# megvii-research/Far3D

Measured on AMD Instinct MI355X. Metric: samples/sec (7-cam frame) end-to-end @ VoV-99 640x960, higher is better.
Workload: dtype bf16x3; 1 GPU; BASELINE configs[1]: 7 cameras 3x640x960, VoV-99, A=1544 queries (644 learned + 644 adaptive + 256 propagated), 2312 self-attn keys, 6 decoder layers, streaming memory on, ego motion on; proposals=topk, fused_rows=True, parallelism=single GPU, weights=seeded random (far3d_amd.weights.init_state_dict, seed 0)

## Files before the change

far3d_amd/csrc/norm.hip:

```cpp
#include "common.hpp"

__device__ __forceinline__ float wave_sum(float v) {
#pragma unroll
  for (int o = 32; o >= 1; o >>= 1) v += __shfl_xor(v, o);
  return v;
}

template <int MAXV>
__global__ __launch_bounds__(256) void layernorm_kernel(const float* __restrict__ x, const float* __restrict__ gamma,
                                                        const float* __restrict__ beta, float* __restrict__ y, int rows,
                                                        int C, int ldx, int ldy, float eps, int act,
                                                        const float* __restrict__ add, int lda, void* __restrict__ y2,
                                                        int ldy2, int y2_dt, void* __restrict__ yb, int ldyb, int yb_dt,
                                                        const int* __restrict__ out_rows) {
  const int lane = threadIdx.x & 63;
  const int row = blockIdx.x * 4 + (threadIdx.x >> 6);
  if (row >= rows) return;
  const int orow = out_rows ? out_rows[row] : row;
  const float* xr = x + (long)row * ldx;
  float4 v[MAXV];
  float s = 0.f;
#pragma unroll
  for (int i = 0; i < MAXV; ++i) {
    const int c = (lane + 64 * i) * 4;
// ... 279 lines not shown
    hipLaunchKernelGGL(ese_apply_kernel<float>, dim3((unsigned)blocks), dim3(256), 0, st, (const float*)x, gate,
                       (const float*)identity, (float*)y, total4, C, HW, ldx, x_img_stride, ldi, i_img_stride, ldy, y_img_stride, chan_sums, N * C);
  else if (dt == FAR3D_DT_BF16_PAIR)
    hipLaunchKernelGGL(ese_apply_kernel<pair_t>, dim3((unsigned)blocks), dim3(256), 0, st, (const pair_t*)x, gate,
                       (const pair_t*)identity, (pair_t*)y, total4, C, HW, ldx, x_img_stride, ldi, i_img_stride, ldy, y_img_stride, chan_sums, N * C);
  else
    hipLaunchKernelGGL(ese_apply_kernel<bf16_t>, dim3((unsigned)blocks), dim3(256), 0, st, (const bf16_t*)x, gate,
                       (const bf16_t*)identity, (bf16_t*)y, total4, C, HW, ldx, x_img_stride, ldi, i_img_stride, ldy, y_img_stride, chan_sums, N * C);
  FAR3D_CHECK_LAUNCH("far3d_ese_nhwc");
  return FAR3D_OK;
}

template <typename T> struct Vec8;
template <> struct Vec8<bf16_t> {
  struct Raw { uint4 a; };
  static __device__ __forceinline__ Raw ldraw(const bf16_t* p) { Raw r; r.a = *reinterpret_cast<const uint4*>(p); return r; }
  static __device__ __forceinline__ void cvt(const Raw& q, float (&v)[8]) {
    const uint4 r = q.a;
    v[0] = __uint_as_float(r.x << 16); v[1] = __uint_as_float(r.x & 0xffff0000u); v[2] = __uint_as_float(r.y << 16); v[3] = __uint_as_float(r.y & 0xffff0000u);
    v[4] = __uint_as_float(r.z << 16); v[5] = __uint_as_float(r.z & 0xffff0000u); v[6] = __uint_as_float(r.w << 16); v[7] = __uint_as_float(r.w & 0xffff0000u);
  }
  static __device__ __forceinline__ void ld(const bf16_t* p, float (&v)[8]) {
    const uint4 r = *reinterpret_cast<const uint4*>(p);
    v[0] = __uint_as_float(r.x << 16); v[1] = __uint_as_float(r.x & 0xffff0000u); v[2] = __uint_as_float(r.y << 16); v[3] = __uint_as_float(r.y & 0xffff0000u);
    v[4] = __uint_as_float(r.z << 16); v[5] = __uint_as_float(r.z & 0xffff0000u); v[6] = __uint_as_float(r.w << 16); v[7] = __uint_as_float(r.w & 0xffff0000u);
  }
  static __device__ __forceinline__ void st(bf16_t* p, const float (&v)[8]) {
    *reinterpret_cast<uint4*>(p) = make_uint4(pack_bf16x2(v[0], v[1]), pack_bf16x2(v[2], v[3]), pack_bf16x2(v[4], v[5]), pack_bf16x2(v[6], v[7]));
  }
  static __device__ __forceinline__ void round(float (&v)[8]) {
#pragma unroll
    for (int e = 0; e < 8; e += 2) { const uint32_t q = pack_bf16x2(v[e], v[e + 1]); v[e] = __uint_as_float(q << 16); v[e + 1] = __uint_as_float(q & 0xffff0000u); }
  }
};
template <> struct Vec8<pair_t> {
  struct Raw { uint4 h, l; };
  static __device__ __forceinline__ Raw ldraw(const pair_t* p) {
    Raw r;
    r.h = *reinterpret_cast<const uint4*>(p);
    r.l = *reinterpret_cast<const uint4*>(reinterpret_cast<const bf16_t*>(p) + 32);
    return r;
  }
  static __device__ __forceinline__ void cvt(const Raw& q, float (&v)[8]) {
    float h[8], l[8];
    Vec8<bf16_t>::Raw a, b;
    a.a = q.h; b.a = q.l;
    Vec8<bf16_t>::cvt(a, h);
    Vec8<bf16_t>::cvt(b, l);
#pragma unroll
    for (int e = 0; e < 8; ++e) v[e] = h[e] + l[e];
  }
  static __device__ __forceinline__ void ld(const pair_t* p, float (&v)[8]) {
    float h[8], l[8];
    Vec8<bf16_t>::ld(reinterpret_cast<const bf16_t*>(p), h);
    Vec8<bf16_t>::ld(reinterpret_cast<const bf16_t*>(p) + 32, l);
#pragma unroll
    for (int e = 0; e < 8; ++e) v[e] = h[e] + l[e];
  }
  static __device__ __forceinline__ void split(const float (&v)[8], uint4& h, uint4& l) {
    uint2 h0, l0, h1, l1;
    split4f(v[0], v[1], v[2], v[3], h0, l0);
    split4f(v[4], v[5], v[6], v[7], h1, l1);
    h = make_uint4(h0.x, h0.y, h1.x, h1.y); l = make_uint4(l0.x, l0.y, l1.x, l1.y);
  }
  static __device__ __forceinline__ void st(pair_t* p, const float (&v)[8]) {
    uint4 h, l;
    split(v, h, l);
    *reinterpret_cast<uint4*>(p) = h;
    *reinterpret_cast<uint4*>(reinterpret_cast<bf16_t*>(p) + 32) = l;
  }
  static __device__ __forceinline__ void round(float (&v)[8]) {
    uint4 h, l;
    split(v, h, l);
    const uint32_t hh[4] = {h.x, h.y, h.z, h.w}, ll[4] = {l.x, l.y, l.z, l.w};
#pragma unroll
    for (int e = 0; e < 4; ++e) {
      v[2 * e] = __uint_as_float(hh[e] << 16) + __uint_as_float(ll[e] << 16);
      v[2 * e + 1] = __uint_as_float(hh[e] & 0xffff0000u) + __uint_as_float(ll[e] & 0xffff0000u);
    }
  }
};

struct EseFusedParams {
  const void* x; const void* idn; void* y; void* pooled;
  const float* gate; long long* sums;
  int N, H, W, C, ldx, ldi, ldy, ldp, Hp, Wp, DB;
  long xs, is, ys, ps;
};

template <typename T, bool POOL>
__global__ __launch_bounds__(256) __attribute__((amdgpu_waves_per_eu(4, 8))) void ese_fused_kernel(EseFusedParams P) {
  const int n = blockIdx.y, tid = threadIdx.x, C = P.C;
  const int b = blockIdx.x, cq = C / 8;
  const int HW = P.H * P.W;
  const int stride = P.DB * 256;
  const int i0 = b * 256 + tid;
  const int cg = i0 % cq, pstep = stride / cq;
  const int co = chan_off<T>(cg * 8);
  const T* x = reinterpret_cast<const T*>(P.x) + (long)n * P.xs + co;
  const T* idn = P.idn ? reinterpret_cast<const T*>(P.idn) + (long)n * P.is + co : nullptr;
  T* y = P.y ? reinterpret_cast<T*>(P.y) + (long)n * P.ys + co : nullptr;
  int pix = i0 / cq;
  float g[8];
  {
    const float4 g0 = *reinterpret_cast<const float4*>(P.gate + (long)n * C + cg * 8), g1 = *reinterpret_cast<const float4*>(P.gate + (long)n * C + cg * 8 + 4);
    g[0] = g0.x; g[1] = g0.y; g[2] = g0.z; g[3] = g0.w; g[4] = g1.x; g[5] = g1.y; g[6] = g1.z; g[7] = g1.w;
  }
  float xv[8], dv[8];
  if (y && pix < HW) {
    Vec8<T>::ld(x + (long)pix * P.ldx, xv);
    if (idn) Vec8<T>::ld(idn + (long)pix * P.ldi, dv);
  }
  for (int i = i0; i < C; i += stride) P.sums[(long)n * C + i] = 0;
  if (y) {
    for (; pix < HW; pix += pstep) {
      const int nxt = pix + pstep;
      float xn[8], dn[8];
      if (nxt < HW) {
        Vec8<T>::ld(x + (long)nxt * P.ldx, xn);
        if (idn) Vec8<T>::ld(idn + (long)nxt * P.ldi, dn);
      }
#pragma unroll
      for (int e = 0; e < 8; ++e) xv[e] = idn ? ese_mul_add(xv[e], g[e], dv[e]) : ese_mul(xv[e], g[e]);
      Vec8<T>::st(y + (long)pix * P.ldy, xv);
#pragma unroll
      for (int e = 0; e < 8; ++e) { xv[e] = xn[e]; dv[e] = dn[e]; }
    }
  }
  if constexpr (POOL) {
    T* pd = reinterpret_cast<T*>(P.pooled) + (long)n * P.ps + co;
    const int HWp = P.Hp * P.Wp;
    for (int q = i0 / cq; q < HWp; q += pstep) {
      const int oy = q / P.Wp, ox = q - oy * P.Wp;
      float m[8];
#pragma unroll
      for (int e = 0; e < 8; ++e) m[e] = -INFINITY;
#pragma unroll 1
      for (int ky = 0; ky < 3; ++ky) {
        const int iy = min(oy * 2 + ky, P.H - 1);
        typename Vec8<T>::Raw tv[3], td[3];
#pragma unroll
        for (int kx = 0; kx < 3; ++kx) {
          const long pp = (long)iy * P.W + min(ox * 2 + kx, P.W - 1);
          tv[kx] = Vec8<T>::ldraw(x + pp * P.ldx);
          if (idn) td[kx] = Vec8<T>::ldraw(idn + pp * P.ldi);
        }
#pragma unroll
        for (int kx = 0; kx < 3; ++kx) {
          float v[8], d[8];
          Vec8<T>::cvt(tv[kx], v);
          if (idn) Vec8<T>::cvt(td[kx], d);
#pragma unroll
          for (int e = 0; e < 8; ++e) v[e] = idn ? ese_mul_add(v[e], g[e], d[e]) : ese_mul(v[e], g[e]);
          Vec8<T>::round(v);
#pragma unroll
          for (int e = 0; e < 8; ++e) m[e] = fmaxf(m[e], v[e]);
        }
      }
      Vec8<T>::st(pd + (long)q * P.ldp, m);
    }
  }
}

extern "C" int far3d_ese_fused_nhwc(const void* x, int dt, const float* fcw, const float* fcb, const void* identity, void* y, void* pooled,
                                    float* gate, int N, int H, int W, int C, int ldx, long x_img_stride, int ldi,
                                    long i_img_stride, int ldy, long y_img_stride, int Hp, int Wp, int ldp, long p_img_stride,
                                    long long* chan_sums, void* stream) {
  FAR3D_CHECK_ARG(x && fcw && fcb && gate && chan_sums && (y || pooled), "far3d_ese_fused_nhwc: null pointer argument (y or pooled must be given)");
  FAR3D_CHECK_ARG(dt == FAR3D_DT_BF16 || dt == FAR3D_DT_BF16_PAIR, "far3d_ese_fused_nhwc: bf16 or pair-stored maps (the fixed-point channel sums describe those)");
  FAR3D_CHECK_ARG(N > 0 && H > 0 && W > 0 && C > 0 && C <= 1024 && C % (dt == FAR3D_DT_BF16_PAIR ? 32 : 8) == 0, "far3d_ese_fused_nhwc: bad sizes (C=%d)", C);
  auto al = [](const void* p) { return ((uintptr_t)p % 16) == 0; };
  FAR3D_CHECK_ARG(al(x) && ldx % 8 == 0 && x_img_stride % 8 == 0 && (!identity || (al(identity) && ldi % 8 == 0 && i_img_stride % 8 == 0)) &&
                  (!y || (al(y) && ldy % 8 == 0 && y_img_stride % 8 == 0)) && (!pooled || (al(pooled) && ldp % 8 == 0 && p_img_stride % 8 == 0)) && al(gate),
                  "far3d_ese_fused_nhwc: pointers and strides must be multiples of 16 bytes");
  if (pooled) {
    int eh = (H - 3 + 1) / 2 + 1; if ((eh - 1) * 2 >= H) --eh;
    int ew = (W - 3 + 1) / 2 + 1; if ((ew - 1) * 2 >= W) --ew;
    FAR3D_CHECK_ARG(Hp == eh && Wp == ew, "far3d_ese_fused_nhwc: pooled size %dx%d != ceil-mode size %dx%d", Hp, Wp, eh, ew);
  }
  hipStream_t st = (hipStream_t)stream;
  hipLaunchKernelGGL(ese_gate_kernel, dim3((C + 15) / 16, N), dim3(256), 0, st, (const float*)nullptr, fcw, fcb, gate, C, 1.f / ((float)H * W), 0,
                     (const long long*)chan_sums);
  EseFusedParams P;
  P.x = x; P.idn = identity; P.y = y; P.pooled = pooled; P.gate = gate; P.sums = chan_sums;
  P.N = N; P.H = H; P.W = W; P.C = C; P.ldx = ldx; P.ldi = ldi; P.ldy = ldy; P.ldp = ldp; P.Hp = Hp; P.Wp = Wp;
  P.xs = x_img_stride; P.is = i_img_stride; P.ys = y_img_stride; P.ps = p_img_stride;
  const int cq = C / 8;
  int unit = 1;
  while ((256 * unit) % cq) ++unit;
  const long items = (long)(y ? H * W : Hp * Wp) * cq;
  long db = (items + 4 * 256 - 1) / (4 * 256);
  if (db > 1200) db = 1200;
  db = (db + unit - 1) / unit * unit;
  P.DB = (int)db;
  dim3 grid((unsigned)P.DB, (unsigned)N);
  if (dt == FAR3D_DT_BF16_PAIR) {
    if (pooled) hipLaunchKernelGGL((ese_fused_kernel<pair_t, true>), grid, dim3(256), 0, st, P);
    else hipLaunchKernelGGL((ese_fused_kernel<pair_t, false>), grid, dim3(256), 0, st, P);
  } else {
    if (pooled) hipLaunchKernelGGL((ese_fused_kernel<bf16_t, true>), grid, dim3(256), 0, st, P);
    else hipLaunchKernelGGL((ese_fused_kernel<bf16_t, false>), grid, dim3(256), 0, st, P);
  }
  FAR3D_CHECK_LAUNCH("far3d_ese_fused_nhwc");
  return FAR3D_OK;
}

__global__ __launch_bounds__(256) void gn_stats_kernel(const float* __restrict__ part, float* __restrict__ stat, int C,
                                                       int groups, float inv_cnt, float eps, int nparts) {
  __shared__ float2 cs[1024];
  const int n = blockIdx.x, cpg = C / groups;
  const float2* src = reinterpret_cast<const float2*>(part) + (long)n * nparts * C;
  float2 sm[4];
  sum_parts<4>(src, nparts, C, threadIdx.x, 256, sm);
#pragma unroll
  for (int j = 0; j < 4; ++j)
    if (threadIdx.x + j * 256 < C) cs[threadIdx.x + j * 256] = sm[j];
  __syncthreads();
  for (int g = threadIdx.x; g < groups; g += 256) {
    float s = 0.f, q = 0.f;
    for (int c = g * cpg; c < (g + 1) * cpg; ++c) { s += cs[c].x; q += cs[c].y; }
    const float mean = s * inv_cnt;
    const float var = fmaxf(q * inv_cnt - mean * mean, 0.f);
    stat[2 * ((long)n * groups + g)] = mean;
    stat[2 * ((long)n * groups + g) + 1] = 1.f / sqrtf(var + eps);
  }
}

template <typename T>
__global__ __launch_bounds__(256) void gn_apply_kernel(const T* __restrict__ x, const float* __restrict__ stat,
                                                       const float* __restrict__ gamma, const float* __restrict__ beta,
                                                       T* __restrict__ y, long total4, int C, int groups, int HW, int relu) {
  const int cq = C / 4, cpg = C / groups;
  for (long i = (long)blockIdx.x * blockDim.x + threadIdx.x; i < total4; i += (long)gridDim.x * blockDim.x) {
    const int c = (int)(i % cq) * 4;
// ... 94 lines not shown
```

far3d_amd/csrc/stem.hip:

```cpp
#include "igemm_kernels.hpp"

__global__ __launch_bounds__(256) __attribute__((amdgpu_waves_per_eu(4, 8))) void stem_conv_kernel(const float* __restrict__ img, const bf16_t* __restrict__ w, const float* __restrict__ bias,
                                                        bf16_t* __restrict__ y, int N, int H, int W, int Ho, int Wo, int ldy, long y_img_stride,
                                                        int tiles_x, int ntiles, int relu) {
  constexpr int RS = 144;
  __shared__ __attribute__((aligned(16))) unsigned char smem[4 * 32 * RS];
  const int lane = threadIdx.x & 63, wv = threadIdx.x >> 6, l31 = lane & 31, hi = lane >> 5;
  unsigned char* my = smem + wv * 32 * RS;
  u32x4_t af[2][2];
#pragma unroll
  for (int i = 0; i < 2; ++i)
#pragma unroll
    for (int h = 0; h < 2; ++h) af[i][h] = *reinterpret_cast<const u32x4_t*>(w + (long)(i * 32 + l31) * 32 + h * 16 + hi * 8);
  int kinfo[16];
#pragma unroll
  for (int s = 0; s < 16; ++s) {
    const int k = (s >> 3) * 16 + hi * 8 + (s & 7);
    const int tap = (k * 11) >> 5, c = k - 3 * tap;
    const int dy = (tap * 11) >> 5, dx = tap - 3 * dy;
    kinfo[s] = ((c * H + dy) * W + dx) | (dy << 24) | (dx << 26) | ((k >= 27 ? 1 : 0) << 28);
  }
  auto gather = [&](int t, float (&v)[16]) __attribute__((always_inline)) {
    const int tx = t % tiles_x, r = t / tiles_x, oy = r % Ho, n = r / Ho;
    const int ox = tx * 32 + l31;
    const int iy0 = 2 * oy - 1, ix0 = 2 * ox - 1;
    const float* base = img + ((long)n * 3 * H + iy0) * W + ix0;
#pragma unroll
    for (int s = 0; s < 16; ++s) {
      const int iy = iy0 + ((kinfo[s] >> 24) & 3), ix = ix0 + ((kinfo[s] >> 26) & 3);
      const bool ok = ox < Wo && !(kinfo[s] >> 28) && iy >= 0 && iy < H && ix >= 0 && ix < W;
      v[s] = ok ? base[kinfo[s] & 0xffffff] : 0.f;
    }
  };
  const int wstride = gridDim.x * 4;
  int t = blockIdx.x * 4 + wv;
  for (; t < ntiles; t += wstride) {
    float cur[16];
    gather(t, cur);
    u32x4_t bf0, bf1;
    bf0.x = pack_bf16x2(cur[0], cur[1]); bf0.y = pack_bf16x2(cur[2], cur[3]); bf0.z = pack_bf16x2(cur[4], cur[5]); bf0.w = pack_bf16x2(cur[6], cur[7]);
    bf1.x = pack_bf16x2(cur[8], cur[9]); bf1.y = pack_bf16x2(cur[10], cur[11]); bf1.z = pack_bf16x2(cur[12], cur[13]); bf1.w = pack_bf16x2(cur[14], cur[15]);
    f32x16_t acc[2];
#pragma unroll
    for (int i = 0; i < 2; ++i) {
#pragma unroll
      for (int r = 0; r < 16; ++r) acc[i][r] = 0.f;
      mma<bf16_t>(acc[i], af[i][0], bf0);
      mma<bf16_t>(acc[i], af[i][1], bf1);
    }
#pragma unroll
    for (int i = 0; i < 2; ++i)
#pragma unroll
      for (int q = 0; q < 4; ++q) {
        const float4 b4 = bias ? *reinterpret_cast<const float4*>(bias + i * 32 + 8 * q + 4 * hi) : make_float4(0.f, 0.f, 0.f, 0.f);
        float v0 = acc[i][4 * q] + b4.x, v1 = acc[i][4 * q + 1] + b4.y, v2 = acc[i][4 * q + 2] + b4.z, v3 = acc[i][4 * q + 3] + b4.w;
        if (relu) { v0 = fmaxf(v0, 0.f); v1 = fmaxf(v1, 0.f); v2 = fmaxf(v2, 0.f); v3 = fmaxf(v3, 0.f); }
        *reinterpret_cast<uint2*>(my + l31 * RS + (i * 32 + 8 * q + 4 * hi) * 2) = make_uint2(pack_bf16x2(v0, v1), pack_bf16x2(v2, v3));
      }
    __builtin_amdgcn_wave_barrier();
    asm volatile("s_waitcnt lgkmcnt(0)" ::: "memory");
    const int tx = t % tiles_x, r = t / tiles_x, oy = r % Ho, n = r / Ho;
    bf16_t* yrow = y + (long)n * y_img_stride + ((long)oy * Wo + tx * 32) * ldy;
#pragma unroll
    for (int it = 0; it < 4; ++it) {
      const int px = it * 8 + (lane >> 3), ch = lane & 7;
      const uint4 v = *reinterpret_cast<const uint4*>(my + px * RS + ch * 16);
      if (tx * 32 + px < Wo) *reinterpret_cast<uint4*>(yrow + (long)px * ldy + ch * 8) = v;
    }
    asm volatile("s_waitcnt lgkmcnt(0)" ::: "memory");
    __builtin_amdgcn_wave_barrier();
  }
}

extern "C" int far3d_stem_conv(const float* img, const void* w, const float* bias, void* y, int N, int H, int W, int ldy, long y_img_stride,
                               int act, void* stream) {
  FAR3D_CHECK_ARG(img && w && y, "far3d_stem_conv: null pointer argument");
  FAR3D_CHECK_ARG(N > 0 && H > 1 && W > 1 && (long)3 * H * W < (1L << 24), "far3d_stem_conv: bad image size N=%d H=%d W=%d (3*H*W < 2^24)", N, H, W);
  FAR3D_CHECK_ARG(act == ACT_NONE || act == ACT_RELU, "far3d_stem_conv: activation none or ReLU");
  FAR3D_CHECK_ARG(((uintptr_t)y % 16) == 0 && ((uintptr_t)w % 16) == 0 && ldy >= 64 && ldy % 8 == 0 && y_img_stride % 8 == 0,
                  "far3d_stem_conv: y / w must be 16-byte aligned, pixel stride a multiple of 8 elements (>= 64)");
  const int Ho = (H - 1) / 2 + 1, Wo = (W - 1) / 2 + 1;
  const int tiles_x = (Wo + 31) / 32, ntiles = N * Ho * tiles_x;
  int blocks = (ntiles + 3) / 4;
  if (blocks > 4096) blocks = 4096;
  hipLaunchKernelGGL(stem_conv_kernel, dim3((unsigned)blocks), dim3(256), 0, (hipStream_t)stream, img, (const bf16_t*)w, bias, (bf16_t*)y, N, H, W, Ho, Wo,
                     ldy, y_img_stride, tiles_x, ntiles, act == ACT_RELU ? 1 : 0);
  FAR3D_CHECK_LAUNCH("far3d_stem_conv");
  return FAR3D_OK;
}
```

far3d_amd/engine.py:

```python
import fnmatch
import functools
import math
import os

import torch
import torch.nn.functional as F

from . import lib as _lib
from . import ops, weights
from .synth import level_starts

PRECISIONS = {
    "bf16": dict(act=torch.bfloat16, value=torch.bfloat16, dec=torch.bfloat16),
    "fp32": dict(act=torch.float32, value=torch.float32, dec=torch.float32),
    "bf16_fp32dec": dict(act=torch.bfloat16, value=torch.bfloat16, dec=torch.float32),
    "bf16_fp32val": dict(act=torch.bfloat16, value=torch.float32, dec=torch.float32),
    "bf16x3": dict(act=torch.bfloat16, pair=True, value=torch.float32, dec=torch.float32, mma="bf16x3", dec_mma=None),
    "bf16x3_all": dict(act=torch.bfloat16, pair=True, value=torch.float32, dec=torch.float32, mma="bf16x3", dec_mma="bf16x3"),
    "bf16x3_2d1": dict(act=torch.bfloat16, pair=True, value=torch.float32, dec=torch.float32, mma="bf16x3", dec_mma=None,
                       single_bf16=("roi[123].*", "depth.*")),
    "bf16x3_f32act": dict(act=torch.float32, value=torch.float32, dec=torch.float32, mma="bf16x3", dec_mma=None),
}


# ... 301 lines not shown
                                     (self.cfg.get("proposal_capacity"), self.cfg["proposal_cap"]))

    def act_from_nchw(self, x):
        y = x.permute(0, 2, 3, 1).contiguous()
        return ops.pair_from_float(y) if self.pair else y.to(self.prec["act"])

    def act_to_nchw(self, y):
        y = ops.pair_to_float(y) if (self.pair and y.dtype == torch.bfloat16) else y.float()
        return y.permute(0, 3, 1, 2).contiguous()

    def _buf(self, key, shape, dtype):
        key = (self._par,) + tuple(key)
        b = self._bufs.get(key)
        if b is None or tuple(b.shape) != tuple(shape) or b.dtype != dtype:
            b = torch.empty(shape, dtype=dtype, device=self.dev)
            self._bufs[key] = b
        return b

    @_with_tile_tables
    def backbone(self, img, keep_stage2=True):
        act, spec, cs, pair = self.prec["act"], self.spec, self.cs, self.pair
        N = img.shape[0]
        Lb = spec["layer_per_block"]
        scratch = self._buf(("ese_scratch",), (ops.ese_scratch_floats(N, max(spec["stage_out_ch"])),), torch.float32)
        esums = None
        if act == torch.bfloat16:
            ek = (self._par, "esums", N)
            esums = self._bufs.get(ek)
            if esums is None:
                esums = self._bufs[ek] = torch.zeros((N, max(spec["stage_out_ch"])), dtype=torch.int64, device=self.dev)
        if esums is not None and not torch.cuda.is_current_stream_capturing():
            esums.zero_()
        egate = self._buf(("ese_gate", N), (N * max(spec["stage_out_ch"]),), torch.float32) if esums is not None else None
        if act == torch.bfloat16 and not pair:
            x = ops.stem_conv(img, self.bb["stem1"], act="relu")
        else:
            x = ops.stem_im2col(img, act, pair=pair)
            x = ops.conv2d_nhwc(x, self.bb["stem1"], act="relu")
        x = ops.conv2d_nhwc(x, self.bb["stem2"], act="relu")
        H, W = self.bb["stem3"].out_hw(x.shape[1], x.shape[2])
        in_ch = spec["stem"][2]
        outs = []
        stage_in = None
        pooled_by_ese = False
        next_cat = None
        for si, blocks in enumerate(self.bb["stages"]):
            sc, oc = spec["stage_conv_ch"][si], spec["stage_out_ch"][si]
            if si > 0:
                Hp, Wp = H, W
                H, W = -(-(Hp - 3) // 2) + 1, -(-(Wp - 3) // 2) + 1
                if (H - 1) * 2 >= Hp:
                    H -= 1
                if (W - 1) * 2 >= Wp:
                    W -= 1
            want_shape = (N, H, W, (in_ch + Lb * sc) * cs)
            if next_cat is not None:
                assert tuple(next_cat.shape) == want_shape, (tuple(next_cat.shape), want_shape)
                cat, next_cat = next_cat, None
            else:
                cat = self._buf(("cat", si, 0), want_shape, act)
            if si == 0:
                ops.conv2d_nhwc(x, self.bb["stem3"], out=cat[..., :in_ch * cs], act="relu")
            elif not pooled_by_ese:
                assert stage_in is not None, "the previous stage's map was skipped (keep_stage2=False) but its eSE pass did not pool it"
                ops.maxpool3x3s2_nhwc(stage_in, out=cat[..., :in_ch * cs], pair=pair)
            pooled_by_ese = False
            cur_in = in_ch
            for bi, blk in enumerate(blocks):
# ... 592 lines not shown
```

far3d_amd/lib.py:

```python
import ctypes
import os

os.environ.setdefault("GPU_MAX_HW_QUEUES", "8")

import torch

_HERE = os.path.dirname(os.path.abspath(__file__))
LIB_PATH = os.path.join(_HERE, "libfar3d_hip.so")

c_int, c_float, c_void_p, c_char_p = ctypes.c_int, ctypes.c_float, ctypes.c_void_p, ctypes.c_char_p
c_long = ctypes.c_long
_p = c_void_p

SIGNATURES = {
    "far3d_last_error": (c_char_p, []),
    "far3d_abi_version": (c_int, []),
    "far3d_device_count": (c_int, []),
    "far3d_device_arch": (c_int, [c_int, c_char_p, c_int]),
    "far3d_msda_forward": (c_int, [_p, c_int, _p, _p, _p, _p, _p] + [c_int] * 7 + [_p]),
    "far3d_aggregate_forward": (c_int, [_p, c_int, _p, _p, _p, _p, _p, _p, _p, _p, c_int] + [c_int] * 7 +
                                [_p, _p, _p, c_float, c_float, c_int, c_int, c_int, _p, _p, c_int, _p, _p]),
    "far3d_conv2d_nhwc": (c_int, [_p, c_int, _p, c_int, _p, _p, c_int] + [c_int] * 5 + [c_long] + [c_int] * 4 +
                          [c_long] + [c_int] * 5 + [_p, c_int, c_int, c_long, c_int, c_int] +
                          [_p, c_int, c_int, c_long, _p, _p, _p, c_int, _p]),
    "far3d_conv2d_nhwc_grouped": (c_int, [_p, c_int, c_int, _p]),
    "far3d_attention_forward": (c_int, [_p, _p, _p, c_int, _p, c_int] + [c_int] * 8 + [c_float, _p, c_int, c_int, _p]),
    "far3d_attention_f32_variant": (c_int, [c_int]),
    "far3d_layernorm": (c_int, [_p, _p, _p, _p, c_int, c_int, c_int, c_int, c_float, c_int, _p, c_int, _p, c_int, c_int, _p, c_int, c_int, _p]),
    "far3d_layernorm_rows": (c_int, [_p, _p, _p, _p, c_int, c_int, c_int, c_int, c_float, c_int, _p, c_int, _p, c_int, c_int, _p, c_int, c_int, _p, _p]),
    "far3d_rowchain_attn_out": (c_int, [_p, c_int, _p, c_int, _p, c_int, _p, _p, _p, _p, _p, _p, c_int, _p, c_int, _p, c_int,
                                        _p, c_int, c_float, _p]),
    "far3d_rowchain_ffn": (c_int, [_p, c_int, _p, c_int, _p, c_int] + [_p] * 12 + [_p, c_int, _p, c_int, _p, c_int, c_int, c_float, _p]),
    "far3d_rowchain_qkv": (c_int, [_p, c_int, _p, c_int, _p, _p, _p, c_int, c_int, _p]),
    "far3d_rowchain_branches": (c_int, [_p, c_int] + [_p] * 10 + [c_int] + [_p] * 6 + [c_int, _p, c_int, _p, c_int, c_int, c_float, _p]),
    "far3d_ese_nhwc": (c_int, [_p, c_int, _p, _p, _p, _p, _p, c_int, c_int, c_int, c_int, c_long, c_int, c_long,
                               c_int, c_long, _p, _p]),
    "far3d_ese_fused_nhwc": (c_int, [_p, c_int, _p, _p, _p, _p, _p, _p, c_int, c_int, c_int, c_int, c_int, c_long, c_int, c_long, c_int, c_long,
                                     c_int, c_int, c_int, c_long, _p, _p]),
    "far3d_cam_embed_chain": (c_int, [_p] * 10 + [c_int, c_int, c_int, c_int, c_float, c_int, _p]),
    "far3d_groupnorm_nhwc": (c_int, [_p, c_int, _p, _p, _p, _p, c_int, c_int, c_int, c_int, c_float, c_int, _p]),
    "far3d_maxpool3x3s2_nhwc": (c_int, [_p, c_int, _p] + [c_int] * 7 + [c_long, _p]),
    "far3d_stem_im2col": (c_int, [_p, _p, c_int, c_int, c_int, c_int, _p]),
    "far3d_stem_conv": (c_int, [_p, _p, _p, _p, c_int, c_int, c_int, c_int, c_long, c_int, _p]),
    "far3d_proposal_select": (c_int, [_p, _p, c_int, c_int, c_int, c_int, _p, _p, _p, _p, _p, _p, c_int, c_float, c_int, _p]),
    "far3d_proposal_gather": (c_int, [_p, c_int, c_int, c_int, _p, _p, _p, _p, c_int, _p, _p, c_int, c_int, c_int, c_int,
                                      c_float, c_float, c_int, _p, _p, c_int, c_int, _p, c_float, _p, _p, _p, _p, c_int, _p, _p, _p]),
    "far3d_proposal_gather_md": (c_int, [_p, c_int, c_int, c_int, _p, _p, _p, _p, c_int, _p, _p, c_int, c_int, c_int, c_int,
                                         c_float, c_float, c_int, _p, _p, c_int, c_int, _p, c_float, _p, _p, _p, _p, c_int,
                                         c_int, c_int, _p, _p, _p]),
    "far3d_proposal_extra_rows": (c_int, [_p, c_int, c_int, c_int, c_int, _p, _p, _p, c_float, c_float, c_int, _p, c_int,
                                          _p, _p, _p, _p, c_int, c_int, _p, _p, _p]),
    "far3d_compact_rows": (c_int, [_p, _p, c_int, c_int, c_int, _p, c_int, _p, _p, _p]),
    "far3d_row_affine_ln": (c_int, [_p, _p, _p, _p, _p] + [c_int] * 6 + [c_float, c_int, _p]),
    "far3d_posemb3d": (c_int, [_p, _p, _p, c_int, _p]),
    "far3d_memory_prepare": (c_int, [_p] * 9 + [c_float, c_int, _p, c_int, c_int, c_int] + [_p] * 9),
    "far3d_head_finalize": (c_int, [_p] * 5 + [c_int] * 4 + [_p, _p, c_int, c_int, _p]),
    "far3d_memory_post_update": (c_int, [_p] * 10 + [c_int] * 4 + [_p] * 6),
    "far3d_add_cast": (c_int, [_p, _p, _p, c_int, _p, c_int, c_int, c_int, c_long, c_long, _p]),
    "far3d_agg_order": (c_int, [_p, _p, _p, c_int, c_int, _p, c_float, c_float, _p, c_int, c_int, c_int, _p, _p, c_int, c_int, c_int, _p, _p, _p]),
    "far3d_agg_tables": (c_int, [_p, _p, c_int, c_int, c_int, _p]),
    "far3d_topk": (c_int, [_p, c_int, c_int, _p, _p, _p]),
    "far3d_decode_topk": (c_int, [_p, _p, c_int, c_int, c_int, c_int, _p, _p, _p, _p, _p, _p, c_long, _p]),
    "far3d_decode_topk_mem": (c_int, [_p, _p, c_int, c_int, c_int, c_int, _p, _p, _p, _p, _p, _p, c_long, _p, c_int, c_int, _p, _p]),
    "far3d_camera_prep": (c_int, [_p, _p, _p, _p, _p, c_int, _p]),
    "far3d_nan_to_num": (c_int, [_p, _p, c_long, _p]),
    "far3d_image_resample_h": (c_int, [_p, c_long, c_int, c_int, _p, _p, _p, c_int, c_int, c_int, c_int, c_int, _p]),
    "far3d_image_resample_v": (c_int, [_p, c_int, c_int, c_int, _p, _p, c_int, c_int, c_int, c_int, c_int, _p, c_int, c_int, c_int,
                                       _p, _p, c_int, _p]),
}

_lib = None


class Far3dHipError(RuntimeError):
    pass

# ... 31 lines not shown
```

far3d_amd/ops.py:

```python
import contextlib
import ctypes
import threading

import numpy as np
import torch

from . import lib as _lib

DT_F32, DT_BF16 = 0, 1
DT_F32_BF16X3 = 2
DT_BF16_PAIR = 3


def pair_from_float(t):
    C = t.shape[-1]
    if C % 32:
        raise ValueError("pair storage needs C %% 32 == 0 (got %d)" % C)
    b = t.float().reshape(t.shape[:-1] + (C // 32, 32))
    hi = b.to(torch.bfloat16)
    lo = (b - hi.float()).to(torch.bfloat16)
    return torch.cat([hi, lo], dim=-1).reshape(t.shape[:-1] + (2 * C,)).contiguous()


def pair_to_float(t):
# ... 767 lines not shown
    _chk(x, "x", ndim=4)
    N, H, W, C = x.shape
    Cs = C
    if pair:
        if x.dtype != torch.bfloat16 or C % 64:
            raise ValueError("maxpool3x3s2_nhwc: pair storage is bf16 with a multiple of 64 stored channels")
        C //= 2
    Ho, Wo = -(-(H - 3) // 2) + 1, -(-(W - 3) // 2) + 1
    if (Ho - 1) * 2 >= H:
        Ho -= 1
    if (Wo - 1) * 2 >= W:
        Wo -= 1
    if out is None:
        out = torch.empty((N, Ho, Wo, Cs), dtype=x.dtype, device=x.device)
    ldy, ys = _nhwc_view(out, "out")
    _lib.check(lib.far3d_maxpool3x3s2_nhwc(_ptr(x), DT_BF16_PAIR if pair else _dt(x), _ptr(out), N, H, W, C, Ho, Wo, ldy, ys, _stream(x)),
               "far3d_maxpool3x3s2_nhwc")
    return out


def stem_im2col(img, out_dtype=torch.bfloat16, out=None, pair=False):
    lib = _lib.require_device()
    _chk(img, "img", torch.float32, 4)
    N, C, H, W = img.shape
    if C != 3:
        raise ValueError("stem_im2col expects 3 input channels")
    Ho, Wo = (H - 1) // 2 + 1, (W - 1) // 2 + 1
    if out is None:
        out = torch.empty((N, Ho, Wo, 64 if pair else 32), dtype=torch.bfloat16 if pair else out_dtype, device=img.device)
    _lib.check(lib.far3d_stem_im2col(_ptr(img), _ptr(out), DT_BF16_PAIR if pair else _dt(out), N, H, W, _stream(img)), "far3d_stem_im2col")
    return out


def stem_conv(img, pc, act="relu", out=None):
    lib = _lib.require_device()
    _chk(img, "img", torch.float32, 4)
    N, C, H, W = img.shape
    if C != 3 or pc.Cout != 64 or pc.Cin != 32 or pc.KH != 1 or pc.w.dtype != torch.bfloat16:
        raise ValueError("stem_conv: 3-channel image and the 64 x 32 bf16 packing of the stem layer")
    Ho, Wo = (H - 1) // 2 + 1, (W - 1) // 2 + 1
    if out is None:
        out = torch.empty((N, Ho, Wo, 64), dtype=torch.bfloat16, device=img.device)
    ldy, ys = _nhwc_view(out, "out")
    _lib.check(lib.far3d_stem_conv(_ptr(img), _ptr(pc.w), _ptr(pc.bias) if pc.bias is not None else None, _ptr(out), N, H, W, ldy, ys,
                                   {None: 0, "relu": 1}[act], _stream(img)), "far3d_stem_conv")
    return out


def _ptr_array(tensors):
    arr = (ctypes.c_void_p * len(tensors))(*[t.data_ptr() for t in tensors])
    return arr


def proposal_select(cls_maps, reg_maps, strides, cap, thr=0.1, topk=False):
    lib = _lib.require_device()
    L = len(cls_maps)
    for t in list(cls_maps) + list(reg_maps):
        _chk(t, "cls/reg map", torch.float32, 4)
    N = cls_maps[0].shape[0]
    hw = [(int(c.shape[1]), int(c.shape[2])) for c in cls_maps]
    S = sum(h * w for h, w in hw)
    dev = cls_maps[0].device
    sw = torch.empty((N, S), dtype=torch.float32, device=dev)
    wgt = torch.empty((N, S), dtype=torch.float32, device=dev)
    sel_idx = torch.empty((N, cap), dtype=torch.int32, device=dev)
    sel_cnt = torch.empty((N,), dtype=torch.int32, device=dev)
    hk, hp = _host_i32([list(x) for x in hw])
    sk, sp = _host_i32(list(strides))
    ca, ra = _ptr_array(cls_maps), _ptr_array(reg_maps)
    _lib.check(lib.far3d_proposal_select(ca, ra, cls_maps[0].shape[3], reg_maps[0].shape[3], N, L, hp, sp, _ptr(sw), _ptr(wgt),
                                         _ptr(sel_idx), _ptr(sel_cnt), cap, float(thr), 1 if topk else 0, _stream(wgt)),
               "far3d_proposal_select")
    return wgt, sel_idx, sel_cnt


def proposal_gather(reg_maps, strides, sel_idx, sel_cnt, weights, depth_logit, depth_stride, depth_cfg, img2lidar,
                    feat, pc_range, score_thr=0.1, out=None, rows_total=0, m_out=None, overflow_out=None):
    lib = _lib.require_device()
# ... 410 lines not shown
```

include/far3d_hip.h:

```cpp
#ifndef FAR3D_HIP_H
#define FAR3D_HIP_H
#include <stdint.h>

#ifdef __cplusplus
extern "C" {
#endif

#define FAR3D_DT_F32 0
#define FAR3D_DT_BF16 1
#define FAR3D_DT_F32_BF16X3 2
#define FAR3D_DT_BF16_PAIR 3
#define FAR3D_SUMS_MAX_PARTS 32
#define FAR3D_SUMS_FRAC_BITS 18
#define FAR3D_SUMS_SCRATCH_FLOATS(N, C) ((long)(N) * (C) * (2 * FAR3D_SUMS_MAX_PARTS + 1))

#define FAR3D_OK 0
#define FAR3D_ERR_ARG (-1)
#define FAR3D_ERR_LAUNCH (-2)
#define FAR3D_ERR_UNSUPPORTED (-3)

const char* far3d_last_error(void);
int far3d_abi_version(void);
int far3d_device_count(void);
int far3d_device_arch(int dev, char* buf, int buflen);
// ... 60 lines not shown
                       const void* w_1, const float* b_1, const void* w_2, const float* b_2,
                       const float* g2, const float* be2, const void* w_qkv, const float* b_qkv,
                       float* out, int ldo, void* qkv, int ldqkv, void* xop, int ldxop, int M, float eps, void* stream);

int far3d_rowchain_qkv(const float* x, int ldx, const float* qpos, int ldq, const void* w_qkv, const float* b_qkv,
                       void* qkv, int ldqkv, int M, void* stream);

int far3d_rowchain_branches(const void* h, int ldh, const void* w_c0, const float* b_c0, const float* g_c0, const float* be_c0,
                            const void* w_c1, const float* b_c1, const float* g_c1, const float* be_c1,
                            const void* w_c2, const float* b_c2, int n_cls, const void* w_r0, const float* b_r0,
                            const void* w_r1, const float* b_r1, const void* w_r2, const float* b_r2, int n_reg,
                            float* cls, int ld_cls, float* reg, int ld_reg, int M, float eps, void* stream);

int far3d_ese_nhwc(const void* x, int dt, const float* fcw, const float* fcb, const void* identity, void* y,
                   float* scratch, int N, int HW, int C, int ldx, long x_img_stride, int ldi, long i_img_stride,
                   int ldy, long y_img_stride, long long* chan_sums, void* stream);

int far3d_ese_fused_nhwc(const void* x, int dt, const float* fcw, const float* fcb, const void* identity, void* y, void* pooled,
                         float* gate, int N, int H, int W, int C, int ldx, long x_img_stride, int ldi,
                         long i_img_stride, int ldy, long y_img_stride, int Hp, int Wp, int ldp, long p_img_stride,
                         long long* chan_sums, void* stream);

int far3d_groupnorm_nhwc(const void* x, int dt, const float* gamma, const float* beta, void* y, float* scratch, int N,
                         int HW, int C, int groups, float eps, int relu, void* stream);

int far3d_maxpool3x3s2_nhwc(const void* x, int dt, void* y, int N, int H, int W, int C, int Ho, int Wo, int ldy,
                            long y_img_stride, void* stream);

int far3d_stem_im2col(const float* img, void* out, int out_dt, int N, int H, int W, void* stream);

int far3d_stem_conv(const float* img, const void* w, const float* bias, void* y, int N, int H, int W, int ldy, long y_img_stride,
                    int act, void* stream);

int far3d_proposal_select(const float* const* cls, const float* const* reg, int ncls, int nreg, int N, int L,
                          const int32_t* level_hw, const int32_t* strides, float* scratch_sw, float* weights, int* sel_idx,
                          int* sel_cnt, int cap, float thr, int mode, void* stream);

int far3d_proposal_gather(const float* const* reg, int nreg, int N, int L, const int32_t* level_hw, const int32_t* strides,
                          const int* sel_idx, const int* sel_cnt, int cap, const float* weights,
                          const float* depth_logit, int hd, int wd, int nd, int depth_stride, float depth_min,
                          float depth_max, int depth_bins, const float* img2lidar, const void* feat, int feat_dt, int C,
                          const float* pc_range, float score_thr, float* ref2d, float* ctx, float* box2d, float* score,
                          int rows_total, int32_t* m_out, int32_t* overflow_out, void* stream);

int far3d_proposal_gather_md(const float* const* reg, int nreg, int N, int L, const int32_t* level_hw, const int32_t* strides,
                             const int* sel_idx, const int* sel_cnt, int cap, const float* weights,
                             const float* depth_logit, int hd, int wd, int nd, int depth_stride, float depth_min,
                             float depth_max, int depth_bins, const float* img2lidar, const void* feat, int feat_dt, int C,
                             const float* pc_range, float score_thr, float* ref2d, float* ctx, float* box2d, float* score,
                             int primary_rows, int topk, int range_min_bin, int32_t* md_flags, int32_t* md_info, void* stream);

int far3d_proposal_extra_rows(const int* sel_cnt, int N, int sel_cap, int primary_rows, int topk, const int32_t* md_flags,
                              const int32_t* md_info, const float* img2lidar, float depth_min, float depth_max, int depth_bins,
                              const float* pc_range, int C, float* ref2d, float* ctx, float* box2d, float* score, int rows_total,
                              int fill_hole, int32_t* m_out, int32_t* overflow_out, void* stream);

int far3d_compact_rows(const float* src, const int32_t* counts, int nblocks, int rows_per_block, int D, float* dst, int dst_rows,
                       int32_t* m_out, int32_t* overflow_out, void* stream);

int far3d_row_affine_ln(const float* x, const float* gamma, const float* beta, const float* add, float* y, int rows, int C,
                        int ldx, int ldg, int lda, int ldy, float eps, int do_ln, void* stream);


int far3d_posemb3d(const float* pos, const float* dim_t128, float* out, int R, void* stream);

int far3d_memory_prepare(const float* emb, const float* ref, const double* ts, const float* pose, const float* velo,
// ... 51 lines not shown
```

Baseline: 73.83 samples/s.

## Tile ESE pooling with row reuse and add fused pair-precision stem conv

```diff
diff --git a/far3d_amd/csrc/norm.hip b/far3d_amd/csrc/norm.hip
--- a/far3d_amd/csrc/norm.hip
+++ b/far3d_amd/csrc/norm.hip
@@ -335,6 +335,12 @@
 #pragma unroll
     for (int e = 0; e < 8; e += 2) { const uint32_t q = pack_bf16x2(v[e], v[e + 1]); v[e] = __uint_as_float(q << 16); v[e + 1] = __uint_as_float(q & 0xffff0000u); }
   }
+  static __device__ __forceinline__ void round_st(bf16_t* p, bool store, float (&v)[8]) {
+    const uint4 q = make_uint4(pack_bf16x2(v[0], v[1]), pack_bf16x2(v[2], v[3]), pack_bf16x2(v[4], v[5]), pack_bf16x2(v[6], v[7]));
+    if (store) *reinterpret_cast<uint4*>(p) = q;
+    Raw r; r.a = q;
+    cvt(r, v);
+  }
 };
 template <> struct Vec8<pair_t> {
   struct Raw { uint4 h, l; };
@@ -382,16 +388,25 @@
       v[2 * e + 1] = __uint_as_float(hh[e] & 0xffff0000u) + __uint_as_float(ll[e] & 0xffff0000u);
     }
   }
+  static __device__ __forceinline__ void round_st(pair_t* p, bool store, float (&v)[8]) {
+    Raw r;
+    split(v, r.h, r.l);
+    if (store) {
+      *reinterpret_cast<uint4*>(p) = r.h;
+      *reinterpret_cast<uint4*>(reinterpret_cast<bf16_t*>(p) + 32) = r.l;
+    }
+    cvt(r, v);
+  }
 };
 
 struct EseFusedParams {
   const void* x; const void* idn; void* y; void* pooled;
   const float* gate; long long* sums;
-  int N, H, W, C, ldx, ldi, ldy, ldp, Hp, Wp, DB;
+  int N, H, W, C, ldx, ldi, ldy, ldp, Hp, Wp, DB, TH;
   long xs, is, ys, ps;
 };
 
-template <typename T, bool POOL>
+template <typename T>
 __global__ __launch_bounds__(256) __attribute__((amdgpu_waves_per_eu(4, 8))) void ese_fused_kernel(EseFusedParams P) {
   const int n = blockIdx.y, tid = threadIdx.x, C = P.C;
   const int b = blockIdx.x, cq = C / 8;
@@ -430,37 +445,81 @@
       for (int e = 0; e < 8; ++e) { xv[e] = xn[e]; dv[e] = dn[e]; }
     }
   }
-  if constexpr (POOL) {
-    T* pd = reinterpret_cast<T*>(P.pooled) + (long)n * P.ps + co;
-    const int HWp = P.Hp * P.Wp;
-    for (int q = i0 / cq; q < HWp; q += pstep) {
-      const int oy = q / P.Wp, ox = q - oy * P.Wp;
-      float m[8];
-#pragma unroll
-      for (int e = 0; e < 8; ++e) m[e] = -INFINITY;
+}
+
+template <typename T, bool IDN>
+__global__ __launch_bounds__(256) void ese_fused_pool_kernel(EseFusedParams P) {
+  constexpr int TW = 2, NC = 2 * TW + 1;
+  const int n = blockIdx.y, C = P.C, cq = C / 8;
+  const int gid = blockIdx.x * 256 + threadIdx.x;
+  for (int i = gid; i < C; i += gridDim.x * 256) P.sums[(long)n * C + i] = 0;
+  const int nstrips = (P.Wp + TW - 1) / TW, nbands = (P.Hp + P.TH - 1) / P.TH;
+  if (gid >= nbands * nstrips * cq) return;
+  const int cg = gid % cq, sb = gid / cq, strip = sb % nstrips, band = sb / nstrips;
+  const int co = chan_off<T>(cg * 8);
+  const T* x = reinterpret_cast<const T*>(P.x) + (long)n * P.xs + co;
+  const T* idn = IDN ? reinterpret_cast<const T*>(P.idn) + (long)n * P.is + co : nullptr;
+  T* y = P.y ? reinterpret_cast<T*>(P.y) + (long)n * P.ys + co : nullptr;
+  T* pd = reinterpret_cast<T*>(P.pooled) + (long)n * P.ps + co;
+  float g[8];
+  {
+    const float4 g0 = *reinterpret_cast<const float4*>(P.gate + (long)n * C + cg * 8), g1 = *reinterpret_cast<const float4*>(P.gate + (long)n * C + cg * 8 + 4);
+    g[0] = g0.x; g[1] = g0.y; g[2] = g0.z; g[3] = g0.w; g[4] = g1.x; g[5] = g1.y; g[6] = g1.z; g[7] = g1.w;
+  }
+  const int ox0 = strip * TW, oy0 = band * P.TH, th = min(P.TH, P.Hp - oy0);
+  const bool last_strip = ox0 + TW >= P.Wp, last_band = oy0 + th >= P.Hp;
+  int ixc[NC];
+  bool own[NC];
+#pragma unroll
+  for (int k = 0; k < NC; ++k) {
+    ixc[k] = min(2 * ox0 + k, P.W - 1);
+    own[k] = 2 * ox0 + k < P.W && (k < 2 * TW || last_strip);
+  }
+  float acc[TW][8];
 #pragma unroll 1
-      for (int ky = 0; ky < 3; ++ky) {
-        const int iy = min(oy * 2 + ky, P.H - 1);
-        typename Vec8<T>::Raw tv[3], td[3];
-#pragma unroll
-        for (int kx = 0; kx < 3; ++kx) {
-          const long pp = (long)iy * P.W + min(ox * 2 + kx, P.W - 1);
-          tv[kx] = Vec8<T>::ldraw(x + pp * P.ldx);
-          if (idn) td[kx] = Vec8<T>::ldraw(idn + pp * P.ldi);
-        }
-#pragma unroll
-        for (int kx = 0; kx < 3; ++kx) {
-          float v[8], d[8];
-          Vec8<T>::cvt(tv[kx], v);
-          if (idn) Vec8<T>::cvt(td[kx], d);
-#pragma unroll
-          for (int e = 0; e < 8; ++e) v[e] = idn ? ese_mul_add(v[e], g[e], d[e]) : ese_mul(v[e], g[e]);
-          Vec8<T>::round(v);
-#pragma unroll
-          for (int e = 0; e < 8; ++e) m[e] = fmaxf(m[e], v[e]);
-        }
+  for (int r = 0; r <= 2 * th; ++r) {
+    const int iy = min(2 * oy0 + r, P.H - 1);
+    const bool own_row = y && 2 * oy0 + r < P.H && (r < 2 * th || last_band);
+    const long rowpix = (long)iy * P.W;
+    typename Vec8<T>::Raw tv[NC], td[NC];
+#pragma unroll
+    for (int k = 0; k < NC; ++k) {
+      tv[k] = Vec8<T>::ldraw(x + (rowpix + ixc[k]) * P.ldx);
+      if constexpr (IDN) td[k] = Vec8<T>::ldraw(idn + (rowpix + ixc[k]) * P.ldi);
+    }
+    float hm[TW][8];
+#pragma unroll
+    for (int k = 0; k < NC; ++k) {
+      float v[8], d[8];
+      Vec8<T>::cvt(tv[k], v);
+      if constexpr (IDN) Vec8<T>::cvt(td[k], d);
+#pragma unroll
+      for (int e = 0; e < 8; ++e) v[e] = IDN ? ese_mul_add(v[e], g[e], d[e]) : ese_mul(v[e], g[e]);
+      Vec8<T>::round_st(y + (rowpix + ixc[k]) * P.ldy, own_row && own[k], v);
+#pragma unroll
+      for (int e = 0; e < 8; ++e) {
+        if (k >= 1) hm[(k - 1) / 2][e] = fmaxf(hm[(k - 1) / 2][e], v[e]);
+        if (k % 2 == 0 && k / 2 < TW) hm[k / 2][e] = v[e];
       }
-      Vec8<T>::st(pd + (long)q * P.ldp, m);
+    }
+    if (r == 0) {
+#pragma unroll
+      for (int j = 0; j < TW; ++j)
+#pragma unroll
+        for (int e = 0; e < 8; ++e) acc[j][e] = hm[j][e];
+      continue;
+    }
+#pragma unroll
+    for (int j = 0; j < TW; ++j)
+#pragma unroll
+      for (int e = 0; e < 8; ++e) acc[j][e] = fmaxf(acc[j][e], hm[j][e]);
+    if (r & 1) continue;
+    const int oy = oy0 + (r >> 1) - 1;
+#pragma unroll
+    for (int j = 0; j < TW; ++j) {
+      if (ox0 + j < P.Wp) Vec8<T>::st(pd + ((long)oy * P.Wp + ox0 + j) * P.ldp, acc[j]);
+#pragma unroll
+      for (int e = 0; e < 8; ++e) acc[j][e] = hm[j][e];
     }
   }
 }
@@ -489,20 +548,35 @@
   P.N = N; P.H = H; P.W = W; P.C = C; P.ldx = ldx; P.ldi = ldi; P.ldy = ldy; P.ldp = ldp; P.Hp = Hp; P.Wp = Wp;
   P.xs = x_img_stride; P.is = i_img_stride; P.ys = y_img_stride; P.ps = p_img_stride;
   const int cq = C / 8;
-  int unit = 1;
-  while ((256 * unit) % cq) ++unit;
-  const long items = (long)(y ? H * W : Hp * Wp) * cq;
-  long db = (items + 4 * 256 - 1) / (4 * 256);
-  if (db > 1200) db = 1200;
-  db = (db + unit - 1) / unit * unit;
-  P.DB = (int)db;
-  dim3 grid((unsigned)P.DB, (unsigned)N);
-  if (dt == FAR3D_DT_BF16_PAIR) {
-    if (pooled) hipLaunchKernelGGL((ese_fused_kernel<pair_t, true>), grid, dim3(256), 0, st, P);
-    else hipLaunchKernelGGL((ese_fused_kernel<pair_t, false>), grid, dim3(256), 0, st, P);
+  if (pooled) {
+    const long per_band = (long)((Wp + 1) / 2) * cq;
+    long nb = 262144 / (per_band * N);
+    if (nb < 1) nb = 1;
+    if (nb > Hp) nb = Hp;
+    P.TH = (int)((Hp + nb - 1) / nb);
+    P.DB = 0;
+    const long items = (long)((Hp + P.TH - 1) / P.TH) * per_band;
+    FAR3D_CHECK_ARG(items < (1L << 30), "far3d_ese_fused_nhwc: map too large");
+    dim3 grid((unsigned)((items + 255) / 256), (unsigned)N);
+    if (dt == FAR3D_DT_BF16_PAIR) {
+      if (identity) hipLaunchKernelGGL((ese_fused_pool_kernel<pair_t, true>), grid, dim3(256), 0, st, P);
+      else hipLaunchKernelGGL((ese_fused_pool_kernel<pair_t, false>), grid, dim3(256), 0, st, P);
+    } else {
+      if (identity) hipLaunchKernelGGL((ese_fused_pool_kernel<bf16_t, true>), grid, dim3(256), 0, st, P);
+      else hipLaunchKernelGGL((ese_fused_pool_kernel<bf16_t, false>), grid, dim3(256), 0, st, P);
+    }
   } else {
-    if (pooled) hipLaunchKernelGGL((ese_fused_kernel<bf16_t, true>), grid, dim3(256), 0, st, P);
-    else hipLaunchKernelGGL((ese_fused_kernel<bf16_t, false>), grid, dim3(256), 0, st, P);
+    int unit = 1;
+    while ((256 * unit) % cq) ++unit;
+    const long items = (long)H * W * cq;
+    long db = (items + 4 * 256 - 1) / (4 * 256);
+    if (db > 1200) db = 1200;
+    db = (db + unit - 1) / unit * unit;
+    P.DB = (int)db;
+    P.TH = 0;
+    dim3 grid((unsigned)P.DB, (unsigned)N);
+    if (dt == FAR3D_DT_BF16_PAIR) hipLaunchKernelGGL((ese_fused_kernel<pair_t>), grid, dim3(256), 0, st, P);
+    else hipLaunchKernelGGL((ese_fused_kernel<bf16_t>), grid, dim3(256), 0, st, P);
   }
   FAR3D_CHECK_LAUNCH("far3d_ese_fused_nhwc");
   return FAR3D_OK;
diff --git a/far3d_amd/csrc/stem.hip b/far3d_amd/csrc/stem.hip
--- a/far3d_amd/csrc/stem.hip
+++ b/far3d_amd/csrc/stem.hip
@@ -1,17 +1,22 @@
 #include "igemm_kernels.hpp"
 
-__global__ __launch_bounds__(256) __attribute__((amdgpu_waves_per_eu(4, 8))) void stem_conv_kernel(const float* __restrict__ img, const bf16_t* __restrict__ w, const float* __restrict__ bias,
+template <bool PAIR>
+__global__ __launch_bounds__(256) __attribute__((amdgpu_waves_per_eu(PAIR ? 3 : 4, 8))) void stem_conv_kernel(const float* __restrict__ img, const bf16_t* __restrict__ w, const float* __restrict__ bias,
                                                         bf16_t* __restrict__ y, int N, int H, int W, int Ho, int Wo, int ldy, long y_img_stride,
                                                         int tiles_x, int ntiles, int relu) {
-  constexpr int RS = 144;
+  constexpr int PL = PAIR ? 2 : 1;
+  constexpr int RS = 64 * 2 * PL + 16;
+  constexpr int WROW = 32 * PL;
   __shared__ __attribute__((aligned(16))) unsigned char smem[4 * 32 * RS];
   const int lane = threadIdx.x & 63, wv = threadIdx.x >> 6, l31 = lane & 31, hi = lane >> 5;
   unsigned char* my = smem + wv * 32 * RS;
-  u32x4_t af[2][2];
+  u32x4_t af[2][2][PL];
 #pragma unroll
   for (int i = 0; i < 2; ++i)
 #pragma unroll
-    for (int h = 0; h < 2; ++h) af[i][h] = *reinterpret_cast<const u32x4_t*>(w + (long)(i * 32 + l31) * 32 + h * 16 + hi * 8);
+    for (int h = 0; h < 2; ++h)
+#pragma unroll
+      for (int pl = 0; pl < PL; ++pl) af[i][h][pl] = *reinterpret_cast<const u32x4_t*>(w + (long)(i * 32 + l31) * WROW + pl * 32 + h * 16 + hi * 8);
   int kinfo[16];
 #pragma unroll
   for (int s = 0; s < 16; ++s) {
@@ -37,16 +42,34 @@
   for (; t < ntiles; t += wstride) {
     float cur[16];
     gather(t, cur);
-    u32x4_t bf0, bf1;
-    bf0.x = pack_bf16x2(cur[0], cur[1]); bf0.y = pack_bf16x2(cur[2], cur[3]); bf0.z = pack_bf16x2(cur[4], cur[5]); bf0.w = pack_bf16x2(cur[6], cur[7]);
-    bf1.x = pack_bf16x2(cur[8], cur[9]); bf1.y = pack_bf16x2(cur[10], cur[11]); bf1.z = pack_bf16x2(cur[12], cur[13]); bf1.w = pack_bf16x2(cur[14], cur[15]);
+    u32x4_t bf[2][PL];
+#pragma unroll
+    for (int h = 0; h < 2; ++h) {
+      uint32_t q[4];
+#pragma unroll
+      for (int e = 0; e < 4; ++e) q[e] = pack_bf16x2(cur[h * 8 + 2 * e], cur[h * 8 + 2 * e + 1]);
+      bf[h][0].x = q[0]; bf[h][0].y = q[1]; bf[h][0].z = q[2]; bf[h][0].w = q[3];
+      if constexpr (PAIR) {
+        uint32_t lq[4];
+#pragma unroll
+        for (int e = 0; e < 4; ++e)
+          lq[e] = pack_bf16x2(cur[h * 8 + 2 * e] - __uint_as_float(q[e] << 16), cur[h * 8 + 2 * e + 1] - __uint_as_float(q[e] & 0xffff0000u));
+        bf[h][1].x = lq[0]; bf[h][1].y = lq[1]; bf[h][1].z = lq[2]; bf[h][1].w = lq[3];
+      }
+    }
     f32x16_t acc[2];
 #pragma unroll
     for (int i = 0; i < 2; ++i) {
 #pragma unroll
       for (int r = 0; r < 16; ++r) acc[i][r] = 0.f;
-      mma<bf16_t>(acc[i], af[i][0], bf0);
-      mma<bf16_t>(acc[i], af[i][1], bf1);
+#pragma unroll
+      for (int h = 0; h < 2; ++h) {
+        if constexpr (PAIR) {
+          mma<bf16_t>(acc[i], af[i][h][1], bf[h][0]);
+          mma<bf16_t>(acc[i], af[i][h][0], bf[h][1]);
+        }
+        mma<bf16_t>(acc[i], af[i][h][0], bf[h][0]);
+      }
     }
 #pragma unroll
     for (int i = 0; i < 2; ++i)
@@ -55,15 +78,24 @@
         const float4 b4 = bias ? *reinterpret_cast<const float4*>(bias + i * 32 + 8 * q + 4 * hi) : make_float4(0.f, 0.f, 0.f, 0.f);
         float v0 = acc[i][4 * q] + b4.x, v1 = acc[i][4 * q + 1] + b4.y, v2 = acc[i][4 * q + 2] + b4.z, v3 = acc[i][4 * q + 3] + b4.w;
         if (relu) { v0 = fmaxf(v0, 0.f); v1 = fmaxf(v1, 0.f); v2 = fmaxf(v2, 0.f); v3 = fmaxf(v3, 0.f); }
-        *reinterpret_cast<uint2*>(my + l31 * RS + (i * 32 + 8 * q + 4 * hi) * 2) = make_uint2(pack_bf16x2(v0, v1), pack_bf16x2(v2, v3));
+        if constexpr (PAIR) {
+          uint2 h2, l2;
+          split4f(v0, v1, v2, v3, h2, l2);
+          unsigned char* d = my + l31 * RS + i * 128 + (8 * q + 4 * hi) * 2;
+          *reinterpret_cast<uint2*>(d) = h2;
+          *reinterpret_cast<uint2*>(d + 64) = l2;
+        } else {
+          *reinterpret_cast<uint2*>(my + l31 * RS + (i * 32 + 8 * q + 4 * hi) * 2) = make_uint2(pack_bf16x2(v0, v1), pack_bf16x2(v2, v3));
+        }
       }
     __builtin_amdgcn_wave_barrier();
     asm volatile("s_waitcnt lgkmcnt(0)" ::: "memory");
     const int tx = t % tiles_x, r = t / tiles_x, oy = r % Ho, n = r / Ho;
     bf16_t* yrow = y + (long)n * y_img_stride + ((long)oy * Wo + tx * 32) * ldy;
+    constexpr int CPP = 8 * PL;
 #pragma unroll
-    for (int it = 0; it < 4; ++it) {
-      const int px = it * 8 + (lane >> 3), ch = lane & 7;
+    for (int it = 0; it < 32 * CPP / 64; ++it) {
+      const int px = it * (64 / CPP) + lane / CPP, ch = lane % CPP;
       const uint4 v = *reinterpret_cast<const uint4*>(my + px * RS + ch * 16);
       if (tx * 32 + px < Wo) *reinterpret_cast<uint4*>(yrow + (long)px * ldy + ch * 8) = v;
     }
@@ -72,19 +104,33 @@
   }
 }
 
-extern "C" int far3d_stem_conv(const float* img, const void* w, const float* bias, void* y, int N, int H, int W, int ldy, long y_img_stride,
-                               int act, void* stream) {
+static int stem_conv_launch(const float* img, const void* w, const float* bias, void* y, int pair, int N, int H, int W, int ldy, long y_img_stride,
+                            int act, void* stream) {
   FAR3D_CHECK_ARG(img && w && y, "far3d_stem_conv: null pointer argument");
   FAR3D_CHECK_ARG(N > 0 && H > 1 && W > 1 && (long)3 * H * W < (1L << 24), "far3d_stem_conv: bad image size N=%d H=%d W=%d (3*H*W < 2^24)", N, H, W);
   FAR3D_CHECK_ARG(act == ACT_NONE || act == ACT_RELU, "far3d_stem_conv: activation none or ReLU");
-  FAR3D_CHECK_ARG(((uintptr_t)y % 16) == 0 && ((uintptr_t)w % 16) == 0 && ldy >= 64 && ldy % 8 == 0 && y_img_stride % 8 == 0,
-                  "far3d_stem_conv: y / w must be 16-byte aligned, pixel stride a multiple of 8 elements (>= 64)");
+  FAR3D_CHECK_ARG(((uintptr_t)y % 16) == 0 && ((uintptr_t)w % 16) == 0 && ldy >= (pair ? 128 : 64) && ldy % 8 == 0 && y_img_stride % 8 == 0,
+                  "far3d_stem_conv: y / w must be 16-byte aligned, pixel stride a multiple of 8 elements (>= 64, pair storage >= 128)");
   const int Ho = (H - 1) / 2 + 1, Wo = (W - 1) / 2 + 1;
   const int tiles_x = (Wo + 31) / 32, ntiles = N * Ho * tiles_x;
   int blocks = (ntiles + 3) / 4;
   if (blocks > 4096) blocks = 4096;
-  hipLaunchKernelGGL(stem_conv_kernel, dim3((unsigned)blocks), dim3(256), 0, (hipStream_t)stream, img, (const bf16_t*)w, bias, (bf16_t*)y, N, H, W, Ho, Wo,
-                     ldy, y_img_stride, tiles_x, ntiles, act == ACT_RELU ? 1 : 0);
+  if (pair)
+    hipLaunchKernelGGL(stem_conv_kernel<true>, dim3((unsigned)blocks), dim3(256), 0, (hipStream_t)stream, img, (const bf16_t*)w, bias, (bf16_t*)y, N, H, W, Ho, Wo,
+                       ldy, y_img_stride, tiles_x, ntiles, act == ACT_RELU ? 1 : 0);
+  else
+    hipLaunchKernelGGL(stem_conv_kernel<false>, dim3((unsigned)blocks), dim3(256), 0, (hipStream_t)stream, img, (const bf16_t*)w, bias, (bf16_t*)y, N, H, W, Ho, Wo,
+                       ldy, y_img_stride, tiles_x, ntiles, act == ACT_RELU ? 1 : 0);
   FAR3D_CHECK_LAUNCH("far3d_stem_conv");
   return FAR3D_OK;
 }
+
+extern "C" int far3d_stem_conv(const float* img, const void* w, const float* bias, void* y, int N, int H, int W, int ldy, long y_img_stride,
+                               int act, void* stream) {
+  return stem_conv_launch(img, w, bias, y, 0, N, H, W, ldy, y_img_stride, act, stream);
+}
+
+extern "C" int far3d_stem_conv_pair(const float* img, const void* w, const float* bias, void* y, int N, int H, int W, int ldy, long y_img_stride,
+                                    int act, void* stream) {
+  return stem_conv_launch(img, w, bias, y, 1, N, H, W, ldy, y_img_stride, act, stream);
+}
diff --git a/far3d_amd/engine.py b/far3d_amd/engine.py
--- a/far3d_amd/engine.py
+++ b/far3d_amd/engine.py
@@ -357,8 +357,8 @@
         if esums is not None and not torch.cuda.is_current_stream_capturing():
             esums.zero_()
         egate = self._buf(("ese_gate", N), (N * max(spec["stage_out_ch"]),), torch.float32) if esums is not None else None
-        if act == torch.bfloat16 and not pair:
-            x = ops.stem_conv(img, self.bb["stem1"], act="relu")
+        if act == torch.bfloat16 and (not pair or self.bb["stem1"].terms == 3):
+            x = ops.stem_conv(img, self.bb["stem1"], act="relu", pair=pair)
         else:
             x = ops.stem_im2col(img, act, pair=pair)
             x = ops.conv2d_nhwc(x, self.bb["stem1"], act="relu")
diff --git a/far3d_amd/lib.py b/far3d_amd/lib.py
--- a/far3d_amd/lib.py
+++ b/far3d_amd/lib.py
@@ -42,6 +42,7 @@
     "far3d_maxpool3x3s2_nhwc": (c_int, [_p, c_int, _p] + [c_int] * 7 + [c_long, _p]),
     "far3d_stem_im2col": (c_int, [_p, _p, c_int, c_int, c_int, c_int, _p]),
     "far3d_stem_conv": (c_int, [_p, _p, _p, _p, c_int, c_int, c_int, c_int, c_long, c_int, _p]),
+    "far3d_stem_conv_pair": (c_int, [_p, _p, _p, _p, c_int, c_int, c_int, c_int, c_long, c_int, _p]),
     "far3d_proposal_select": (c_int, [_p, _p, c_int, c_int, c_int, c_int, _p, _p, _p, _p, _p, _p, c_int, c_float, c_int, _p]),
     "far3d_proposal_gather": (c_int, [_p, c_int, c_int, c_int, _p, _p, _p, _p, c_int, _p, _p, c_int, c_int, c_int, c_int,
                                       c_float, c_float, c_int, _p, _p, c_int, c_int, _p, c_float, _p, _p, _p, _p, c_int, _p, _p, _p]),
diff --git a/far3d_amd/ops.py b/far3d_amd/ops.py
--- a/far3d_amd/ops.py
+++ b/far3d_amd/ops.py
@@ -823,18 +823,23 @@
     return out
 
 
-def stem_conv(img, pc, act="relu", out=None):
+def stem_conv(img, pc, act="relu", out=None, pair=False):
     lib = _lib.require_device()
     _chk(img, "img", torch.float32, 4)
     N, C, H, W = img.shape
     if C != 3 or pc.Cout != 64 or pc.Cin != 32 or pc.KH != 1 or pc.w.dtype != torch.bfloat16:
         raise ValueError("stem_conv: 3-channel image and the 64 x 32 bf16 packing of the stem layer")
+    if pair != (pc.w_code == DT_F32_BF16X3) or (pair and pc.terms != 3):
+        raise ValueError("stem_conv: pair storage takes the pre-split (bf16x3) packing with its three split products, plain bf16 the bf16 one")
     Ho, Wo = (H - 1) // 2 + 1, (W - 1) // 2 + 1
     if out is None:
-        out = torch.empty((N, Ho, Wo, 64), dtype=torch.bfloat16, device=img.device)
+        out = torch.empty((N, Ho, Wo, 128 if pair else 64), dtype=torch.bfloat16, device=img.device)
+    elif out.shape[3] != (128 if pair else 64):
+        raise ValueError("stem_conv: out holds %d stored channels, the layer writes %d" % (out.shape[3], 128 if pair else 64))
     ldy, ys = _nhwc_view(out, "out")
-    _lib.check(lib.far3d_stem_conv(_ptr(img), _ptr(pc.w), _ptr(pc.bias) if pc.bias is not None else None, _ptr(out), N, H, W, ldy, ys,
-                                   {None: 0, "relu": 1}[act], _stream(img)), "far3d_stem_conv")
+    fn = lib.far3d_stem_conv_pair if pair else lib.far3d_stem_conv
+    _lib.check(fn(_ptr(img), _ptr(pc.w), _ptr(pc.bias) if pc.bias is not None else None, _ptr(out), N, H, W, ldy, ys,
+                  {None: 0, "relu": 1}[act], _stream(img)), "far3d_stem_conv")
     return out
 
 
diff --git a/include/far3d_hip.h b/include/far3d_hip.h
--- a/include/far3d_hip.h
+++ b/include/far3d_hip.h
@@ -116,6 +116,9 @@
 int far3d_stem_conv(const float* img, const void* w, const float* bias, void* y, int N, int H, int W, int ldy, long y_img_stride,
                     int act, void* stream);
 
+int far3d_stem_conv_pair(const float* img, const void* w, const float* bias, void* y, int N, int H, int W, int ldy, long y_img_stride,
+                         int act, void* stream);
+
 int far3d_proposal_select(const float* const* cls, const float* const* reg, int ncls, int nreg, int N, int L,
                           const int32_t* level_hw, const int32_t* strides, float* scratch_sw, float* weights, int* sel_idx,
                           int* sel_cnt, int cap, float thr, int mode, void* stream);
```

Result: no change. 74.46 samples/s, median of 6 (+0.9%).
